# sanazkaviani/3d-latent-diffusion-model

Measured on AMD Instinct MI355X. Metric: UNet denoising steps/sec (bf16, 1x4x24x24x24 latent; whole job = sum over GPUs), higher is better.
Workload: dtype bf16

## Files before the change

3d-latent-diffusion-model_amd/csrc/attention.h:

```cpp
#pragma once
#include "common.h"

struct AttnParams {
    const bf16_t* qkv; bf16_t* out;
    int B, N, C, heads; float scale;
    float* lse;
    int d;
};

template <int S, int QW, bool DB, int D = 64>
__global__ __launch_bounds__(64 * QW * S) void attn_fwd_kernel(const AttnParams p) {
    constexpr int KT = 64;
    constexpr int NSL = (D + 63) / 64, DS = D < 64 ? D : 64;
    constexpr int K2 = DS / 32, NDT = DS / 16, CH = DS / 8;
    constexpr int IMG = KT * 128;
    constexpr int TILE = 2 * NSL * IMG;
    constexpr int GT = 64 * QW;
    constexpr int NIT = (KT * CH * NSL) / GT;
    static_assert(S == 1 || D == 64, "the in-workgroup key split is built for D = 64");
    static_assert((KT * CH * NSL) % GT == 0, "staging must divide evenly");
    extern __shared__ __attribute__((aligned(16))) char smem_all[];

    const int tid = threadIdx.x % GT, lane = tid & 63, wave = tid >> 6, grp = threadIdx.x / GT;
    char* smem = smem_all + grp * (DB ? 2 : 1) * TILE;
    const int fr = lane & 15, fg = lane >> 4;
    const int b = blockIdx.z, head = blockIdx.y;
    const int q0 = blockIdx.x * (16 * QW) + wave * 16;
    const int ld = 3 * p.C;
    const bf16_t* base = p.qkv + (size_t)b * p.N * ld;
    const int hoff = head * D;

    bf16x8 qf[NSL][K2];
    {
        int qr = q0 + fr; if (qr >= p.N) qr = p.N - 1;
#pragma unroll
        for (int sl = 0; sl < NSL; ++sl)
#pragma unroll
            for (int k2 = 0; k2 < K2; ++k2)
                qf[sl][k2] = *reinterpret_cast<const bf16x8*>(base + (size_t)qr * ld + hoff + sl * 64 + k2 * 32 + 8 * fg);
    }

    f32x4 ot[NSL][NDT];
#pragma unroll
    for (int sl = 0; sl < NSL; ++sl)
#pragma unroll
        for (int i = 0; i < NDT; ++i) ot[sl][i] = (f32x4){0.f, 0.f, 0.f, 0.f};
    float mrun = -INFINITY, lrun = 0.f;
    const float cexp = p.scale * 1.44269504088896340736f;

    u32x4 kreg[NIT], vreg[NIT];
    auto stage_load = [&](int k0) {
#pragma unroll
        for (int it = 0; it < NIT; ++it) {
            const int idx = tid + it * GT;
            const int sl = idx / (KT * CH), rem = idx - sl * (KT * CH);
            const int row = rem / CH, ch = rem - row * CH;
            int kr = k0 + row; if (kr >= p.N) kr = p.N - 1;
            const bf16_t* tok = base + (size_t)kr * ld + hoff + sl * 64 + ch * 8;
            kreg[it] = *reinterpret_cast<const u32x4*>(tok + p.C);
            vreg[it] = *reinterpret_cast<const u32x4*>(tok + 2 * p.C);
        }
    };
    auto stage_write = [&](char* ks, char* vs) {
#pragma unroll
        for (int it = 0; it < NIT; ++it) {
            const int idx = tid + it * GT;
            const int sl = idx / (KT * CH), rem = idx - sl * (KT * CH);
            const int row = rem / CH, ch = rem - row * CH;
            *reinterpret_cast<u32x4*>(ks + sl * IMG + row * 128 + ((ch ^ ((row >> 1) & 7)) << 4)) = kreg[it];
            *reinterpret_cast<u32x4*>(vs + sl * IMG + row * 128 + ((ch ^ (((row >> 1) & 3) << 1)) << 4)) = vreg[it];
        }
    };

    const int ntile = (p.N + KT - 1) / KT;
    const int nrounds = (ntile + S - 1) / S;
    stage_load(grp * KT);
#pragma unroll
    for (int sl = 0; sl < NSL; ++sl)
#pragma unroll
        for (int k2 = 0; k2 < K2; ++k2) asm volatile("" :: "v"(qf[sl][k2]));
    stage_write(smem, smem + NSL * IMG);
    __syncthreads();
    for (int it = 0; it < nrounds; ++it) {
        const int t = it * S + grp;
        const int k0 = t * KT;
        const char* ks = smem + (DB ? (it & 1) * TILE : 0);
        const char* vs = ks + NSL * IMG;
        stage_load(k0 + S * KT);
        if (t < ntile) {
        f32x4 st[4];
#pragma unroll
        for (int j = 0; j < 4; ++j) {
            st[j] = (f32x4){0.f, 0.f, 0.f, 0.f};
            const int row = j * 16 + fr;
#pragma unroll
            for (int sl = 0; sl < NSL; ++sl)
#pragma unroll
                for (int k2 = 0; k2 < K2; ++k2) {
                    const int c = k2 * 4 + fg;
                    const bf16x8 kf = *reinterpret_cast<const bf16x8*>(ks + sl * IMG + row * 128 + ((c ^ ((row >> 1) & 7)) << 4));
                    st[j] = __builtin_amdgcn_mfma_f32_16x16x32_bf16(kf, qf[sl][k2], st[j], 0, 0, 0);
                }
        }
        if (k0 + KT > p.N) {
#pragma unroll
            for (int j = 0; j < 4; ++j)
#pragma unroll
                for (int r = 0; r < 4; ++r)
                    if (k0 + 16 * j + 4 * fg + r >= p.N) st[j][r] = -INFINITY;
        }
        float tmax = fmaxf(fmaxf(fmaxf(st[0][0], st[0][1]), fmaxf(st[0][2], st[0][3])), fmaxf(fmaxf(st[1][0], st[1][1]), fmaxf(st[1][2], st[1][3])));
        tmax = fmaxf(tmax, fmaxf(fmaxf(fmaxf(st[2][0], st[2][1]), fmaxf(st[2][2], st[2][3])), fmaxf(fmaxf(st[3][0], st[3][1]), fmaxf(st[3][2], st[3][3]))));
        tmax = fmaxf(tmax, __shfl_xor(tmax, 16, 64));
        tmax = fmaxf(tmax, __shfl_xor(tmax, 32, 64));
        const float mnew = fmaxf(mrun, tmax);
        const float alpha = __builtin_amdgcn_exp2f((mrun - mnew) * cexp);
        const float mc = -mnew * cexp;
        mrun = mnew;
        float psum = 0.f;
        bf16x8 pf[2];
#pragma unroll
        for (int h = 0; h < 2; ++h) {
            float pv[8];
#pragma unroll
            for (int e = 0; e < 8; ++e) {
                const float pe = __builtin_amdgcn_exp2f(fmaf(st[2 * h + (e >> 2)][e & 3], cexp, mc));
                psum += pe;
                pv[e] = pe;
            }
            u32x4 pk;
#pragma unroll
            for (int e = 0; e < 4; ++e) pk[e] = pack2bf(pv[2 * e], pv[2 * e + 1]);
            pf[h] = *reinterpret_cast<bf16x8*>(&pk);
        }
        lrun = lrun * alpha + psum;
        if (__builtin_amdgcn_ballot_w64(alpha != 1.0f)) {
#pragma unroll
            for (int sl = 0; sl < NSL; ++sl)
#pragma unroll
                for (int dt = 0; dt < NDT; ++dt) {
#pragma unroll
                    for (int r = 0; r < 4; ++r) ot[sl][dt][r] *= alpha;
                }
        }
        typedef __attribute__((ext_vector_type(4))) short s16x4;
        typedef __attribute__((address_space(3))) s16x4* lds_s16x4_t;
        const int tq = fr >> 2, tp = fr & 3;
#pragma unroll
        for (int sl = 0; sl < NSL; ++sl)
#pragma unroll
        for (int dt = 0; dt < NDT; ++dt) {
#pragma unroll
            for (int h = 0; h < 2; ++h) {
                const int rlo = (2 * h) * 16 + 4 * fg + tq, rhi = rlo + 16;
                const char* alo = vs + sl * IMG + rlo * 128 + ((dt ^ ((rlo >> 1) & 3)) << 5) + tp * 8;
                const char* ahi = vs + sl * IMG + rhi * 128 + ((dt ^ ((rhi >> 1) & 3)) << 5) + tp * 8;
                const s16x4 lo = __builtin_amdgcn_ds_read_tr16_b64_v4i16((lds_s16x4_t)alo);
                const s16x4 hi = __builtin_amdgcn_ds_read_tr16_b64_v4i16((lds_s16x4_t)ahi);
                const bf16x8 vf = {lo[0], lo[1], lo[2], lo[3], hi[0], hi[1], hi[2], hi[3]};
                ot[sl][dt] = __builtin_amdgcn_mfma_f32_16x16x32_bf16(vf, pf[h], ot[sl][dt], 0, 0, 0);
            }
        }
        }
        if constexpr (!DB) __syncthreads();
        {
            char* nk = smem + (DB ? ((it + 1) & 1) * TILE : 0);
            stage_write(nk, nk + NSL * IMG);
        }
        __syncthreads();
    }
    lrun += __shfl_xor(lrun, 16, 64);
    lrun += __shfl_xor(lrun, 32, 64);
    if constexpr (S > 1) {
        float* xo = reinterpret_cast<float*>(smem_all) + (size_t)(grp * QW + wave) * (1024 + 32);
        if (grp > 0) {
#pragma unroll
            for (int dt = 0; dt < NDT; ++dt) *reinterpret_cast<f32x4*>(xo + (dt * 64 + lane) * 4) = ot[0][dt];
            if (fg == 0) { xo[1024 + fr] = mrun; xo[1040 + fr] = lrun; }
        }
        __syncthreads();
        if (grp > 0) return;
#pragma unroll
        for (int g = 1; g < S; ++g) {
            const float* xg = reinterpret_cast<const float*>(smem_all) + (size_t)(g * QW + wave) * (1024 + 32);
            const float mg = xg[1024 + fr], lg = xg[1040 + fr];
            const float mnew = fmaxf(mrun, mg);
            const float a0 = __builtin_amdgcn_exp2f((mrun - mnew) * cexp), a1 = __builtin_amdgcn_exp2f((mg - mnew) * cexp);
            lrun = lrun * a0 + lg * a1;
            mrun = mnew;
#pragma unroll
            for (int dt = 0; dt < NDT; ++dt) {
                const f32x4 og = *reinterpret_cast<const f32x4*>(xg + (dt * 64 + lane) * 4);
#pragma unroll
                for (int r = 0; r < 4; ++r) ot[0][dt][r] = ot[0][dt][r] * a0 + og[r] * a1;
            }
        }
    }
    const float inv = 1.0f / lrun;
    const int qr = q0 + fr;
    if (p.lse && qr < p.N && fg == 0) p.lse[((size_t)b * p.heads + head) * p.N + qr] = mrun * p.scale + __logf(lrun);
    if (qr < p.N) {
        bf16_t* orow = p.out + ((size_t)b * p.N + qr) * p.C + hoff;
#pragma unroll
        for (int sl = 0; sl < NSL; ++sl)
#pragma unroll
        for (int dt = 0; dt < NDT; ++dt) {
            u32x2 o;
            o[0] = pack2bf(ot[sl][dt][0] * inv, ot[sl][dt][1] * inv);
            o[1] = pack2bf(ot[sl][dt][2] * inv, ot[sl][dt][3] * inv);
            *reinterpret_cast<u32x2*>(orow + sl * 64 + dt * 16 + 4 * fg) = o;
        }
    }
}

template <int D>
static inline hipError_t launch_attn_fwd_d(const AttnParams& p, hipStream_t s) {
    constexpr int LDS = 2 * 2 * ((D + 63) / 64) * 64 * 128;
    static bool once_tab[32] = {}; bool& once = attr_flag(once_tab);
    if (!once) {
        hipError_t e = hipFuncSetAttribute(reinterpret_cast<const void*>(&attn_fwd_kernel<1, 4, true, D>), hipFuncAttributeMaxDynamicSharedMemorySize, LDS);
        if (e != hipSuccess) return e;
        once = true;
    }
    hipLaunchKernelGGL((attn_fwd_kernel<1, 4, true, D>), dim3((p.N + 63) / 64, p.heads, p.B), dim3(256), LDS, s, p);
    return hipGetLastError();
}
static inline hipError_t launch_attn_fwd(const AttnParams& p, hipStream_t s) {
    if (p.d == 32) return launch_attn_fwd_d<32>(p, s);
    if (p.d == 128) return launch_attn_fwd_d<128>(p, s);
    if (p.d == 256) return launch_attn_fwd_d<256>(p, s);
    if (p.d != 64) return hipErrorInvalidValue;
    static bool once_tab[32] = {}; bool& once = attr_flag(once_tab);
    if (!once) {
        hipError_t e = hipFuncSetAttribute(reinterpret_cast<const void*>(&attn_fwd_kernel<4, 4, true>), hipFuncAttributeMaxDynamicSharedMemorySize, 4 * 32768);
        if (e == hipSuccess) e = hipFuncSetAttribute(reinterpret_cast<const void*>(&attn_fwd_kernel<8, 2, false>), hipFuncAttributeMaxDynamicSharedMemorySize, 8 * 16384);
        if (e != hipSuccess) return e;
        once = true;
    }
    if (p.N >= 1024 && (long)((p.N + 63) / 64) * p.heads * p.B < 128)
        hipLaunchKernelGGL((attn_fwd_kernel<8, 2, false>), dim3((p.N + 31) / 32, p.heads, p.B), dim3(1024), 8 * 16384, s, p);
    else if (p.N > 3 * 64) hipLaunchKernelGGL((attn_fwd_kernel<4, 4, true>), dim3((p.N + 63) / 64, p.heads, p.B), dim3(1024), 4 * 32768, s, p);
    else hipLaunchKernelGGL((attn_fwd_kernel<1, 4, true>), dim3((p.N + 63) / 64, p.heads, p.B), dim3(256), 32768, s, p);
    return hipGetLastError();
}


struct AttnBwdParams {
    const bf16_t* qkv; const bf16_t* o; const bf16_t* d_o; const float* lse;
    float* delta;
    bf16_t* dqkv;
    int B, N, C, heads; float scale;
    int d;
};

__global__ __launch_bounds__(256) void attn_delta_kernel(const AttnBwdParams p) {
    const long idx = (long)blockIdx.x * 256 + threadIdx.x;
    const int cpd = p.d >> 3;
    const long total = (long)p.B * p.N * p.heads * cpd;
    float s = 0.f;
    long tok = 0; int head = 0;
    if (idx < total) {
        const int ch = (int)(idx % cpd);
        const long th = idx / cpd;
        head = (int)(th % p.heads); tok = th / p.heads;
        const u32x4 a = *reinterpret_cast<const u32x4*>(p.o + tok * p.C + head * p.d + ch * 8);
        const u32x4 b = *reinterpret_cast<const u32x4*>(p.d_o + tok * p.C + head * p.d + ch * 8);
#pragma unroll
        for (int k = 0; k < 4; ++k)
            s += __uint_as_float(a[k] << 16) * __uint_as_float(b[k] << 16) +
                 __uint_as_float(a[k] & 0xffff0000u) * __uint_as_float(b[k] & 0xffff0000u);
    }
    for (int o = 1; o < cpd; o <<= 1) s += __shfl_xor(s, o, 64);
    if (idx < total && (idx % cpd) == 0) {
        const long bb = tok / p.N, i = tok - bb * p.N;
        p.delta[((size_t)bb * p.heads + head) * p.N + i] = s;
    }
}

typedef __attribute__((ext_vector_type(4))) short attn_s16x4;
typedef __attribute__((address_space(3))) attn_s16x4* attn_lds_s16x4_t;

__device__ __forceinline__ int attn_row_off(int row, int ch) { return row * 128 + ((ch ^ ((row >> 1) & 7)) << 4); }
__device__ __forceinline__ int attn_tr_off(int row, int ch) { return row * 128 + ((ch ^ (((row >> 1) & 3) << 1)) << 4); }
__device__ __forceinline__ bf16x8 attn_tr_frag(const char* img, int dt, int h, int fr, int fg) {
    const int tq = fr >> 2, tp = fr & 3;
    const int rlo = (2 * h) * 16 + 4 * fg + tq, rhi = rlo + 16;
    const attn_s16x4 lo = __builtin_amdgcn_ds_read_tr16_b64_v4i16((attn_lds_s16x4_t)(img + rlo * 128 + ((dt ^ ((rlo >> 1) & 3)) << 5) + tp * 8));
    const attn_s16x4 hi = __builtin_amdgcn_ds_read_tr16_b64_v4i16((attn_lds_s16x4_t)(img + rhi * 128 + ((dt ^ ((rhi >> 1) & 3)) << 5) + tp * 8));
    return (bf16x8){lo[0], lo[1], lo[2], lo[3], hi[0], hi[1], hi[2], hi[3]};
}

template <int D>
__global__ __launch_bounds__(256) void attn_bwd_dq_kernel(const AttnBwdParams p) {
    constexpr int KT = 64;
    constexpr int NSL = (D + 63) / 64, DS = D < 64 ? D : 64, K2 = DS / 32, NDT = DS / 16, CH = DS / 8, IMG = KT * 128;
    constexpr int NIT = (KT * CH * NSL) / 256;
    extern __shared__ __attribute__((aligned(16))) char smem[];
    char* k_row = smem; char* k_tr = smem + NSL * IMG; char* v_row = smem + 2 * NSL * IMG;
    const int tid = threadIdx.x, lane = tid & 63, wave = tid >> 6;
    const int fr = lane & 15, fg = lane >> 4;
    const int b = blockIdx.z, head = blockIdx.y;
    const int q0 = blockIdx.x * 64 + wave * 16;
    const int ld = 3 * p.C, hoff = head * D;
    const bf16_t* base = p.qkv + (size_t)b * p.N * ld;
    int qr = q0 + fr; const bool qok = qr < p.N; if (!qok) qr = p.N - 1;
    bf16x8 qf[NSL][K2], dof[NSL][K2];
#pragma unroll
    for (int sl = 0; sl < NSL; ++sl)
#pragma unroll
    for (int k2 = 0; k2 < K2; ++k2) {
        qf[sl][k2] = *reinterpret_cast<const bf16x8*>(base + (size_t)qr * ld + hoff + sl * 64 + k2 * 32 + 8 * fg);
        dof[sl][k2] = *reinterpret_cast<const bf16x8*>(p.d_o + ((size_t)b * p.N + qr) * p.C + hoff + sl * 64 + k2 * 32 + 8 * fg);
    }
    const float lse = p.lse[((size_t)b * p.heads + head) * p.N + qr];
    const float dlt = p.delta[((size_t)b * p.heads + head) * p.N + qr];
    f32x4 dq[NSL][NDT];
#pragma unroll
    for (int sl = 0; sl < NSL; ++sl)
#pragma unroll
    for (int i = 0; i < NDT; ++i) dq[sl][i] = (f32x4){0.f, 0.f, 0.f, 0.f};
    const int ntile = (p.N + KT - 1) / KT;
    u32x4 kreg[NIT], vreg[NIT];
    auto stage_load = [&](int k0) {
#pragma unroll
        for (int it = 0; it < NIT; ++it) {
            const int idx = tid + it * 256, sl = idx / (KT * CH), rem = idx - sl * (KT * CH), row = rem / CH, ch = rem - row * CH;
            int kr = k0 + row; if (kr >= p.N) kr = p.N - 1;
            const bf16_t* tok = base + (size_t)kr * ld + hoff + sl * 64 + ch * 8;
            kreg[it] = *reinterpret_cast<const u32x4*>(tok + p.C);
            vreg[it] = *reinterpret_cast<const u32x4*>(tok + 2 * p.C);
        }
    };
    stage_load(0);
#pragma unroll
    for (int sl = 0; sl < NSL; ++sl)
#pragma unroll
        for (int k2 = 0; k2 < K2; ++k2) asm volatile("" :: "v"(qf[sl][k2]), "v"(dof[sl][k2]));
    asm volatile("" :: "v"(lse), "v"(dlt));
    for (int t = 0; t < ntile; ++t) {
        const int k0 = t * KT;
        __syncthreads();
#pragma unroll
        for (int it = 0; it < NIT; ++it) {
            const int idx = tid + it * 256, sl = idx / (KT * CH), rem = idx - sl * (KT * CH), row = rem / CH, ch = rem - row * CH;
            *reinterpret_cast<u32x4*>(k_row + sl * IMG + attn_row_off(row, ch)) = kreg[it];
            *reinterpret_cast<u32x4*>(k_tr + sl * IMG + attn_tr_off(row, ch)) = kreg[it];
            *reinterpret_cast<u32x4*>(v_row + sl * IMG + attn_row_off(row, ch)) = vreg[it];
        }
        __syncthreads();
        stage_load(k0 + KT);
        bf16x8 dsf[2];
        f32x4 st[4], dp[4];
#pragma unroll
        for (int j = 0; j < 4; ++j) {
            st[j] = (f32x4){0.f, 0.f, 0.f, 0.f}; dp[j] = (f32x4){0.f, 0.f, 0.f, 0.f};
            const int row = j * 16 + fr;
#pragma unroll
            for (int sl = 0; sl < NSL; ++sl)
#pragma unroll
            for (int k2 = 0; k2 < K2; ++k2) {
                const bf16x8 kf = *reinterpret_cast<const bf16x8*>(k_row + sl * IMG + attn_row_off(row, k2 * 4 + fg));
                const bf16x8 vf = *reinterpret_cast<const bf16x8*>(v_row + sl * IMG + attn_row_off(row, k2 * 4 + fg));
                st[j] = __builtin_amdgcn_mfma_f32_16x16x32_bf16(kf, qf[sl][k2], st[j], 0, 0, 0);
                dp[j] = __builtin_amdgcn_mfma_f32_16x16x32_bf16(vf, dof[sl][k2], dp[j], 0, 0, 0);
            }
        }
#pragma unroll
        for (int h = 0; h < 2; ++h) {
            float dsv[8];
#pragma unroll
            for (int e = 0; e < 8; ++e) {
                const int j = 2 * h + (e >> 2), r = e & 3;
                const int key = k0 + 16 * j + 4 * fg + r;
                const float pe = (key < p.N) ? __expf(st[j][r] * p.scale - lse) : 0.f;
                dsv[e] = pe * (dp[j][r] - dlt);
            }
            u32x4 pk;
#pragma unroll
            for (int e = 0; e < 4; ++e) pk[e] = pack2bf(dsv[2 * e], dsv[2 * e + 1]);
            dsf[h] = *reinterpret_cast<bf16x8*>(&pk);
        }
#pragma unroll
        for (int sl = 0; sl < NSL; ++sl)
#pragma unroll
        for (int dt = 0; dt < NDT; ++dt)
#pragma unroll
            for (int h = 0; h < 2; ++h)
                dq[sl][dt] = __builtin_amdgcn_mfma_f32_16x16x32_bf16(attn_tr_frag(k_tr + sl * IMG, dt, h, fr, fg), dsf[h], dq[sl][dt], 0, 0, 0);
    }
    if (qok) {
        bf16_t* orow = p.dqkv + ((size_t)b * p.N + qr) * ld + hoff;
#pragma unroll
        for (int sl = 0; sl < NSL; ++sl)
#pragma unroll
        for (int dt = 0; dt < NDT; ++dt) {
            u32x2 o;
            o[0] = pack2bf(dq[sl][dt][0] * p.scale, dq[sl][dt][1] * p.scale);
            o[1] = pack2bf(dq[sl][dt][2] * p.scale, dq[sl][dt][3] * p.scale);
            *reinterpret_cast<u32x2*>(orow + sl * 64 + dt * 16 + 4 * fg) = o;
        }
    }
}

template <int D>
__global__ __launch_bounds__(256) void attn_bwd_dkv_kernel(const AttnBwdParams p) {
    constexpr int QT = 64;
    constexpr int NSL = (D + 63) / 64, DS = D < 64 ? D : 64, K2 = DS / 32, NDT = DS / 16, CH = DS / 8, IMG = QT * 128;
    constexpr int NIT = (QT * CH * NSL) / 256;
    extern __shared__ __attribute__((aligned(16))) char smem[];
    char* q_row = smem; char* q_tr = smem + NSL * IMG; char* do_row = smem + 2 * NSL * IMG; char* do_tr = smem + 3 * NSL * IMG;
    float* s_lse = reinterpret_cast<float*>(smem + 4 * NSL * IMG); float* s_dlt = s_lse + QT;
    const int tid = threadIdx.x, lane = tid & 63, wave = tid >> 6;
    const int fr = lane & 15, fg = lane >> 4;
    const int b = blockIdx.z, head = blockIdx.y;
    const int kv0 = blockIdx.x * 64 + wave * 16;
    const int ld = 3 * p.C, hoff = head * D;
    const bf16_t* base = p.qkv + (size_t)b * p.N * ld;
    int kr = kv0 + fr; const bool kok = kr < p.N; if (!kok) kr = p.N - 1;
    bf16x8 kf[NSL][K2], vf[NSL][K2];
#pragma unroll
    for (int sl = 0; sl < NSL; ++sl)
#pragma unroll
    for (int k2 = 0; k2 < K2; ++k2) {
        kf[sl][k2] = *reinterpret_cast<const bf16x8*>(base + (size_t)kr * ld + p.C + hoff + sl * 64 + k2 * 32 + 8 * fg);
        vf[sl][k2] = *reinterpret_cast<const bf16x8*>(base + (size_t)kr * ld + 2 * p.C + hoff + sl * 64 + k2 * 32 + 8 * fg);
    }
    f32x4 dk[NSL][NDT], dv[NSL][NDT];
#pragma unroll
    for (int sl = 0; sl < NSL; ++sl)
#pragma unroll
    for (int i = 0; i < NDT; ++i) { dk[sl][i] = (f32x4){0.f, 0.f, 0.f, 0.f}; dv[sl][i] = (f32x4){0.f, 0.f, 0.f, 0.f}; }
    const int ntile = (p.N + QT - 1) / QT;
    u32x4 qreg[NIT], oreg[NIT]; float lreg = 0.f, dreg = 0.f;
    auto stage_load = [&](int q0) {
#pragma unroll
        for (int it = 0; it < NIT; ++it) {
            const int idx = tid + it * 256, sl = idx / (QT * CH), rem = idx - sl * (QT * CH), row = rem / CH, ch = rem - row * CH;
            int qr = q0 + row; if (qr >= p.N) qr = p.N - 1;
            qreg[it] = *reinterpret_cast<const u32x4*>(base + (size_t)qr * ld + hoff + sl * 64 + ch * 8);
            oreg[it] = *reinterpret_cast<const u32x4*>(p.d_o + ((size_t)b * p.N + qr) * p.C + hoff + sl * 64 + ch * 8);
        }
        {
            int qr = q0 + (tid & (QT - 1)); const bool ok = qr < p.N; if (!ok) qr = p.N - 1;
            const float l = p.lse[((size_t)b * p.heads + head) * p.N + qr];
            lreg = ok ? l : INFINITY;
            dreg = p.delta[((size_t)b * p.heads + head) * p.N + qr];
        }
    };
    stage_load(0);
#pragma unroll
    for (int sl = 0; sl < NSL; ++sl)
#pragma unroll
        for (int k2 = 0; k2 < K2; ++k2) asm volatile("" :: "v"(kf[sl][k2]), "v"(vf[sl][k2]));
    for (int t = 0; t < ntile; ++t) {
        const int q0 = t * QT;
        __syncthreads();
#pragma unroll
        for (int it = 0; it < NIT; ++it) {
            const int idx = tid + it * 256, sl = idx / (QT * CH), rem = idx - sl * (QT * CH), row = rem / CH, ch = rem - row * CH;
            *reinterpret_cast<u32x4*>(q_row + sl * IMG + attn_row_off(row, ch)) = qreg[it];
            *reinterpret_cast<u32x4*>(q_tr + sl * IMG + attn_tr_off(row, ch)) = qreg[it];
            *reinterpret_cast<u32x4*>(do_row + sl * IMG + attn_row_off(row, ch)) = oreg[it];
            *reinterpret_cast<u32x4*>(do_tr + sl * IMG + attn_tr_off(row, ch)) = oreg[it];
        }
        if (tid < QT) { s_lse[tid] = lreg; s_dlt[tid] = dreg; }
        __syncthreads();
        stage_load(q0 + QT);
        f32x4 st[4], dp[4];
#pragma unroll
        for (int j = 0; j < 4; ++j) {
            st[j] = (f32x4){0.f, 0.f, 0.f, 0.f}; dp[j] = (f32x4){0.f, 0.f, 0.f, 0.f};
            const int row = j * 16 + fr;
#pragma unroll
            for (int sl = 0; sl < NSL; ++sl)
#pragma unroll
            for (int k2 = 0; k2 < K2; ++k2) {
                const bf16x8 qf = *reinterpret_cast<const bf16x8*>(q_row + sl * IMG + attn_row_off(row, k2 * 4 + fg));
                const bf16x8 of = *reinterpret_cast<const bf16x8*>(do_row + sl * IMG + attn_row_off(row, k2 * 4 + fg));
                st[j] = __builtin_amdgcn_mfma_f32_16x16x32_bf16(qf, kf[sl][k2], st[j], 0, 0, 0);
                dp[j] = __builtin_amdgcn_mfma_f32_16x16x32_bf16(of, vf[sl][k2], dp[j], 0, 0, 0);
            }
        }
        bf16x8 pf[2], dsf[2];
#pragma unroll
        for (int h = 0; h < 2; ++h) {
            float pv[8], dsv[8];
#pragma unroll
            for (int e = 0; e < 8; ++e) {
                const int j = 2 * h + (e >> 2), r = e & 3;
                const int ql = 16 * j + 4 * fg + r;
                const float pe = __expf(st[j][r] * p.scale - s_lse[ql]);
                pv[e] = pe; dsv[e] = pe * (dp[j][r] - s_dlt[ql]);
            }
            u32x4 pk, dk_;
#pragma unroll
            for (int e = 0; e < 4; ++e) { pk[e] = pack2bf(pv[2 * e], pv[2 * e + 1]); dk_[e] = pack2bf(dsv[2 * e], dsv[2 * e + 1]); }
            pf[h] = *reinterpret_cast<bf16x8*>(&pk); dsf[h] = *reinterpret_cast<bf16x8*>(&dk_);
        }
#pragma unroll
        for (int sl = 0; sl < NSL; ++sl)
#pragma unroll
        for (int dt = 0; dt < NDT; ++dt)
#pragma unroll
            for (int h = 0; h < 2; ++h) {
                dv[sl][dt] = __builtin_amdgcn_mfma_f32_16x16x32_bf16(attn_tr_frag(do_tr + sl * IMG, dt, h, fr, fg), pf[h], dv[sl][dt], 0, 0, 0);
                dk[sl][dt] = __builtin_amdgcn_mfma_f32_16x16x32_bf16(attn_tr_frag(q_tr + sl * IMG, dt, h, fr, fg), dsf[h], dk[sl][dt], 0, 0, 0);
            }
    }
    if (kok) {
        bf16_t* orow = p.dqkv + ((size_t)b * p.N + kr) * ld + hoff;
#pragma unroll
        for (int sl = 0; sl < NSL; ++sl)
#pragma unroll
        for (int dt = 0; dt < NDT; ++dt) {
            u32x2 o;
            o[0] = pack2bf(dk[sl][dt][0] * p.scale, dk[sl][dt][1] * p.scale); o[1] = pack2bf(dk[sl][dt][2] * p.scale, dk[sl][dt][3] * p.scale);
            *reinterpret_cast<u32x2*>(orow + p.C + sl * 64 + dt * 16 + 4 * fg) = o;
            o[0] = pack2bf(dv[sl][dt][0], dv[sl][dt][1]); o[1] = pack2bf(dv[sl][dt][2], dv[sl][dt][3]);
            *reinterpret_cast<u32x2*>(orow + 2 * p.C + sl * 64 + dt * 16 + 4 * fg) = o;
        }
    }
}

template <int D>
static inline hipError_t launch_attn_bwd_d(const AttnBwdParams& p, hipStream_t s) {
    constexpr int NSL = (D + 63) / 64;
    constexpr int LDS_DQ = 3 * NSL * 64 * 128, LDS_DKV = 4 * NSL * 64 * 128 + 2 * 64 * 4;
    static bool once_tab[32] = {}; bool& once = attr_flag(once_tab);
    if (!once) {
        hipError_t e = hipFuncSetAttribute(reinterpret_cast<const void*>(&attn_bwd_dq_kernel<D>), hipFuncAttributeMaxDynamicSharedMemorySize, LDS_DQ);
        if (e == hipSuccess) e = hipFuncSetAttribute(reinterpret_cast<const void*>(&attn_bwd_dkv_kernel<D>), hipFuncAttributeMaxDynamicSharedMemorySize, LDS_DKV);
        if (e != hipSuccess) return e;
        once = true;
    }
    const long dthreads = (long)p.B * p.N * p.heads * (D / 8);
    hipLaunchKernelGGL(attn_delta_kernel, dim3((unsigned)((dthreads + 255) / 256)), dim3(256), 0, s, p);
    hipLaunchKernelGGL(attn_bwd_dq_kernel<D>, dim3((p.N + 63) / 64, p.heads, p.B), dim3(256), LDS_DQ, s, p);
    hipLaunchKernelGGL(attn_bwd_dkv_kernel<D>, dim3((p.N + 63) / 64, p.heads, p.B), dim3(256), LDS_DKV, s, p);
    return hipGetLastError();
}
static inline hipError_t launch_attn_bwd(const AttnBwdParams& p, hipStream_t s) {
    switch (p.d) {
        case 32: return launch_attn_bwd_d<32>(p, s);
        case 64: return launch_attn_bwd_d<64>(p, s);
        case 128: return launch_attn_bwd_d<128>(p, s);
        case 256: return launch_attn_bwd_d<256>(p, s);
    }
    return hipErrorInvalidValue;
}
```

Before: 515.7.

## Add DMA-to-LDS ring-buffered attention forward kernel for long low-occupancy sequences

Result: no change. 520.7 (median of 6 runs) (+1.0%).

```diff
diff --git a/3d-latent-diffusion-model_amd/csrc/attention.h b/3d-latent-diffusion-model_amd/csrc/attention.h
--- a/3d-latent-diffusion-model_amd/csrc/attention.h
+++ b/3d-latent-diffusion-model_amd/csrc/attention.h
@@ -213,6 +213,253 @@
     }
 }
 
+constexpr __host__ __device__ int attn_dma_swz(bool v_img, int row) { return v_img ? ((row >> 1) & 3) << 1 : (row >> 1) & 7; }
+constexpr __host__ __device__ int attn_dma_src_chunk(bool v_img, int row, int slot) { return slot ^ attn_dma_swz(v_img, row); }
+constexpr bool attn_dma_map_ok(bool v_img) {
+    for (int row = 0; row < 64; ++row) {
+        unsigned seen = 0;
+        for (int slot = 0; slot < 8; ++slot) {
+            const int ch = attn_dma_src_chunk(v_img, row, slot);
+            if (ch < 0 || ch > 7) return false;
+            seen |= 1u << ch;
+            const int rd = v_img ? (ch ^ (((row >> 1) & 3) << 1)) : (ch ^ ((row >> 1) & 7));
+            if (rd != slot) return false;
+        }
+        if (seen != 0xffu) return false;
+    }
+    return true;
+}
+static_assert(attn_dma_map_ok(false) && attn_dma_map_ok(true), "slot -> source map must be a bijection and the inverse of the read-side swizzle");
+
+typedef __attribute__((ext_vector_type(4))) short attn_dma_s16x4;
+__device__ __forceinline__ attn_dma_s16x4 attn_dma_read_tr(unsigned lds_addr) {
+    attn_dma_s16x4 v;
+    asm volatile("ds_read_b64_tr_b16 %0, %1" : "=v"(v) : "v"(lds_addr));
+    return v;
+}
+
+template <int S, int QW, int R>
+__global__ __launch_bounds__(64 * QW * S) void attn_fwd_dma_kernel(const AttnParams p) {
+#if defined(__HIP_DEVICE_COMPILE__)
+    constexpr int KT = 64, IMG = KT * 128, TILE = 2 * IMG, GT = 64 * QW;
+    constexpr int PW = 16 / QW;
+    constexpr unsigned OOB = 0x80000000u;
+    static_assert(QW == 2 || QW == 4, "16 pieces per tile are dealt evenly to the group's waves");
+    static_assert(R >= 2 && (R & (R - 1)) == 0 && (R - 1) * PW <= 63, "ring depth: a power of two; vmcnt is a 6-bit counter");
+    static_assert(S * R * TILE <= 160 * 1024 && S * QW * (1024 + 32) * 4 <= S * R * TILE, "LDS budget; the merge area reuses the rings");
+    typedef __attribute__((address_space(3))) void* lds_ptr_t;
+    extern __shared__ __attribute__((aligned(16))) char smem_all[];
+    KSTAMP_BEGIN(8);
+
+    const int tid = threadIdx.x % GT, lane = tid & 63;
+    const int wave = __builtin_amdgcn_readfirstlane(tid >> 6), grp = __builtin_amdgcn_readfirstlane(threadIdx.x / GT);
+    char* smem = smem_all + grp * (R * TILE);
+    const int fr = lane & 15, fg = lane >> 4;
+    const int b = blockIdx.z, head = blockIdx.y;
+    const int q0 = blockIdx.x * (16 * QW) + wave * 16;
+    const int ld = 3 * p.C;
+    const int hoff = head * 64;
+    const int ntile = (p.N + KT - 1) / KT;
+    const int nrounds = (ntile + S - 1) / S;
+
+    bf16x8 qf[2];
+    {
+        int qr = q0 + fr; if (qr >= p.N) qr = p.N - 1;
+        const bf16_t* qrow = p.qkv + ((size_t)b * p.N + qr) * ld + hoff;
+#pragma unroll
+        for (int k2 = 0; k2 < 2; ++k2) qf[k2] = *reinterpret_cast<const bf16x8*>(qrow + k2 * 32 + 8 * fg);
+    }
+
+    const __amdgpu_buffer_rsrc_t rs = __builtin_amdgcn_make_buffer_rsrc((void*)p.qkv, 0, (int)((unsigned)(p.B * p.N) * (unsigned)ld * 2u), 0x00020000);
+    const unsigned ld2 = (unsigned)ld * 2u, tok0 = (unsigned)(b * p.N);
+    int c_row[PW]; unsigned c_col[PW];
+#pragma unroll
+    for (int j = 0; j < PW; ++j) {
+        const int pc = wave * PW + j;
+        const bool v_img = pc >= 8;
+        const int row = (pc & 7) * 8 + (lane >> 3);
+        c_row[j] = row;
+        c_col[j] = (unsigned)((v_img ? 2 : 1) * p.C + hoff + attn_dma_src_chunk(v_img, row, lane & 7) * 8) * 2u;
+    }
+    auto issue = [&](const int i) {
+        const int t = i * S + grp, k0 = t * KT;
+        char* dst = smem + (i & (R - 1)) * TILE + wave * (PW * 1024);
+        const unsigned oob = t < ntile ? 0u : OOB;
+#pragma unroll
+        for (int j = 0; j < PW; ++j) {
+            int kr = k0 + c_row[j]; if (kr >= p.N) kr = p.N - 1;
+            const unsigned vo = ((tok0 + (unsigned)kr) * ld2 + c_col[j]) | oob;
+            __builtin_amdgcn_raw_ptr_buffer_load_lds(rs, (lds_ptr_t)(dst + j * 1024), 16, vo, 0, 0, 0);
+        }
+    };
+#pragma unroll
+    for (int i = 0; i < R - 1; ++i) issue(i);
+#pragma unroll
+    for (int k2 = 0; k2 < 2; ++k2) asm volatile("" :: "v"(qf[k2]));
+    KSTAMP(1);
+
+    f32x4 ot[4];
+#pragma unroll
+    for (int i = 0; i < 4; ++i) ot[i] = (f32x4){0.f, 0.f, 0.f, 0.f};
+    float mrun = -INFINITY, lrun = 0.f;
+    const float cexp = p.scale * 1.44269504088896340736f;
+
+    int k_off[4][2];
+#pragma unroll
+    for (int j = 0; j < 4; ++j)
+#pragma unroll
+        for (int k2 = 0; k2 < 2; ++k2) {
+            const int row = j * 16 + fr, c = k2 * 4 + fg;
+            k_off[j][k2] = row * 128 + ((c ^ ((row >> 1) & 7)) << 4);
+        }
+    unsigned v_lo[4][2], v_hi[4][2];
+    {
+        const int tq = fr >> 2, tp = fr & 3;
+        const unsigned sbase = (unsigned)(size_t)(const __attribute__((address_space(3))) char*)smem + IMG;
+#pragma unroll
+        for (int dt = 0; dt < 4; ++dt)
+#pragma unroll
+            for (int h = 0; h < 2; ++h) {
+                const int rlo = (2 * h) * 16 + 4 * fg + tq, rhi = rlo + 16;
+                v_lo[dt][h] = sbase + rlo * 128 + ((dt ^ ((rlo >> 1) & 3)) << 5) + tp * 8;
+                v_hi[dt][h] = sbase + rhi * 128 + ((dt ^ ((rhi >> 1) & 3)) << 5) + tp * 8;
+            }
+    }
+
+    for (int it = 0; it < nrounds; ++it) {
+        asm volatile("s_waitcnt vmcnt(%0)" ::"n"((R - 2) * PW) : "memory");
+        asm volatile("s_waitcnt lgkmcnt(0)" ::: "memory");
+        __builtin_amdgcn_s_barrier();
+        asm volatile("" ::: "memory");
+        __builtin_amdgcn_sched_barrier(0);
+        if (it == 0) KSTAMP(2);
+        issue(it + R - 1);
+        const int t = it * S + grp, k0 = t * KT;
+        if (t < ntile) {
+            const int soff = (it & (R - 1)) * TILE;
+            const char* ks = smem + soff;
+            f32x4 st[4];
+#pragma unroll
+            for (int j = 0; j < 4; ++j) {
+                st[j] = (f32x4){0.f, 0.f, 0.f, 0.f};
+#pragma unroll
+                for (int k2 = 0; k2 < 2; ++k2) {
+                    const bf16x8 kf = *reinterpret_cast<const bf16x8*>(ks + k_off[j][k2]);
+                    st[j] = __builtin_amdgcn_mfma_f32_16x16x32_bf16(kf, qf[k2], st[j], 0, 0, 0);
+                }
+            }
+            attn_dma_s16x4 vl[4][2], vh[4][2];
+#pragma unroll
+            for (int dt = 0; dt < 4; ++dt)
+#pragma unroll
+                for (int h = 0; h < 2; ++h) {
+                    vl[dt][h] = attn_dma_read_tr(v_lo[dt][h] + soff);
+                    vh[dt][h] = attn_dma_read_tr(v_hi[dt][h] + soff);
+                }
+            if (k0 + KT > p.N) {
+#pragma unroll
+                for (int j = 0; j < 4; ++j)
+#pragma unroll
+                    for (int r = 0; r < 4; ++r)
+                        if (k0 + 16 * j + 4 * fg + r >= p.N) st[j][r] = -INFINITY;
+            }
+            float tmax = fmaxf(fmaxf(fmaxf(st[0][0], st[0][1]), fmaxf(st[0][2], st[0][3])), fmaxf(fmaxf(st[1][0], st[1][1]), fmaxf(st[1][2], st[1][3])));
+            tmax = fmaxf(tmax, fmaxf(fmaxf(fmaxf(st[2][0], st[2][1]), fmaxf(st[2][2], st[2][3])), fmaxf(fmaxf(st[3][0], st[3][1]), fmaxf(st[3][2], st[3][3]))));
+            tmax = fmaxf(tmax, __shfl_xor(tmax, 16, 64));
+            tmax = fmaxf(tmax, __shfl_xor(tmax, 32, 64));
+            const float mnew = fmaxf(mrun, tmax);
+            const float alpha = __builtin_amdgcn_exp2f((mrun - mnew) * cexp);
+            const float mc = -mnew * cexp;
+            mrun = mnew;
+            float psum = 0.f;
+            bf16x8 pf[2];
+#pragma unroll
+            for (int h = 0; h < 2; ++h) {
+                float pv[8];
+#pragma unroll
+                for (int e = 0; e < 8; ++e) {
+                    const float pe = __builtin_amdgcn_exp2f(fmaf(st[2 * h + (e >> 2)][e & 3], cexp, mc));
+                    psum += pe;
+                    pv[e] = pe;
+                }
+                u32x4 pk;
+#pragma unroll
+                for (int e = 0; e < 4; ++e) pk[e] = pack2bf(pv[2 * e], pv[2 * e + 1]);
+                pf[h] = *reinterpret_cast<bf16x8*>(&pk);
+            }
+            lrun = lrun * alpha + psum;
+            if (__builtin_amdgcn_ballot_w64(alpha != 1.0f)) {
+#pragma unroll
+                for (int dt = 0; dt < 4; ++dt)
+#pragma unroll
+                    for (int r = 0; r < 4; ++r) ot[dt][r] *= alpha;
+            }
+            asm volatile("s_waitcnt lgkmcnt(0)"
+                         : "+v"(vl[0][0]), "+v"(vl[0][1]), "+v"(vl[1][0]), "+v"(vl[1][1]), "+v"(vl[2][0]), "+v"(vl[2][1]), "+v"(vl[3][0]), "+v"(vl[3][1]),
+                           "+v"(vh[0][0]), "+v"(vh[0][1]), "+v"(vh[1][0]), "+v"(vh[1][1]), "+v"(vh[2][0]), "+v"(vh[2][1]), "+v"(vh[3][0]), "+v"(vh[3][1])
+                         :: "memory");
+#pragma unroll
+            for (int dt = 0; dt < 4; ++dt)
+#pragma unroll
+                for (int h = 0; h < 2; ++h) {
+                    const bf16x8 vf = {vl[dt][h][0], vl[dt][h][1], vl[dt][h][2], vl[dt][h][3], vh[dt][h][0], vh[dt][h][1], vh[dt][h][2], vh[dt][h][3]};
+                    ot[dt] = __builtin_amdgcn_mfma_f32_16x16x32_bf16(vf, pf[h], ot[dt], 0, 0, 0);
+                }
+        }
+    }
+    asm volatile("s_waitcnt vmcnt(0) lgkmcnt(0)" ::: "memory");
+    KSTAMP(3);
+    lrun += __shfl_xor(lrun, 16, 64);
+    lrun += __shfl_xor(lrun, 32, 64);
+    if constexpr (S > 1) {
+        __syncthreads();
+        float* xo = reinterpret_cast<float*>(smem_all) + (size_t)(grp * QW + wave) * (1024 + 32);
+        if (grp > 0) {
+#pragma unroll
+            for (int dt = 0; dt < 4; ++dt) *reinterpret_cast<f32x4*>(xo + (dt * 64 + lane) * 4) = ot[dt];
+            if (fg == 0) { xo[1024 + fr] = mrun; xo[1040 + fr] = lrun; }
+        }
+        __syncthreads();
+        if (grp > 0) return;
+#pragma unroll
+        for (int g = 1; g < S; ++g) {
+            const float* xg = reinterpret_cast<const float*>(smem_all) + (size_t)(g * QW + wave) * (1024 + 32);
+            const float mg = xg[1024 + fr], lg = xg[1040 + fr];
+            const float mnew = fmaxf(mrun, mg);
+            const float a0 = __builtin_amdgcn_exp2f((mrun - mnew) * cexp), a1 = __builtin_amdgcn_exp2f((mg - mnew) * cexp);
+            lrun = lrun * a0 + lg * a1;
+            mrun = mnew;
+#pragma unroll
+            for (int dt = 0; dt < 4; ++dt) {
+                const f32x4 og = *reinterpret_cast<const f32x4*>(xg + (dt * 64 + lane) * 4);
+#pragma unroll
+                for (int r = 0; r < 4; ++r) ot[dt][r] = ot[dt][r] * a0 + og[r] * a1;
+            }
+        }
+    }
+    KSTAMP(4);
+    const float inv = 1.0f / lrun;
+    const int qr = q0 + fr;
+    if (p.lse && qr < p.N && fg == 0) p.lse[((size_t)b * p.heads + head) * p.N + qr] = mrun * p.scale + __logf(lrun);
+    if (qr < p.N) {
+        bf16_t* orow = p.out + ((size_t)b * p.N + qr) * p.C + hoff;
+#pragma unroll
+        for (int dt = 0; dt < 4; ++dt) {
+            u32x2 o;
+            o[0] = pack2bf(ot[dt][0] * inv, ot[dt][1] * inv);
+            o[1] = pack2bf(ot[dt][2] * inv, ot[dt][3] * inv);
+            *reinterpret_cast<u32x2*>(orow + dt * 16 + 4 * fg) = o;
+        }
+    }
+    KSTAMP_DRAIN(5);
+#endif
+}
+
+template <int S, int QW, int R>
+static inline void launch_attn_fwd_dma(const AttnParams& p, hipStream_t s) {
+    hipLaunchKernelGGL((attn_fwd_dma_kernel<S, QW, R>), dim3((p.N + 16 * QW - 1) / (16 * QW), p.heads, p.B), dim3(64 * QW * S), S * R * 16384, s, p);
+}
+
 template <int D>
 static inline hipError_t launch_attn_fwd_d(const AttnParams& p, hipStream_t s) {
     constexpr int LDS = 2 * 2 * ((D + 63) / 64) * 64 * 128;
@@ -234,12 +481,27 @@
     if (!once) {
         hipError_t e = hipFuncSetAttribute(reinterpret_cast<const void*>(&attn_fwd_kernel<4, 4, true>), hipFuncAttributeMaxDynamicSharedMemorySize, 4 * 32768);
         if (e == hipSuccess) e = hipFuncSetAttribute(reinterpret_cast<const void*>(&attn_fwd_kernel<8, 2, false>), hipFuncAttributeMaxDynamicSharedMemorySize, 8 * 16384);
+        if (e == hipSuccess) e = hipFuncSetAttribute(reinterpret_cast<const void*>(&attn_fwd_dma_kernel<4, 2, 2>), hipFuncAttributeMaxDynamicSharedMemorySize, 8 * 16384);
+#ifdef LDM_EXPERIMENTS
+        if (e == hipSuccess) e = hipFuncSetAttribute(reinterpret_cast<const void*>(&attn_fwd_dma_kernel<2, 4, 4>), hipFuncAttributeMaxDynamicSharedMemorySize, 8 * 16384);
+        if (e == hipSuccess) e = hipFuncSetAttribute(reinterpret_cast<const void*>(&attn_fwd_dma_kernel<1, 4, 8>), hipFuncAttributeMaxDynamicSharedMemorySize, 8 * 16384);
+#endif
         if (e != hipSuccess) return e;
         once = true;
     }
-    if (p.N >= 1024 && (long)((p.N + 63) / 64) * p.heads * p.B < 128)
-        hipLaunchKernelGGL((attn_fwd_kernel<8, 2, false>), dim3((p.N + 31) / 32, p.heads, p.B), dim3(1024), 8 * 16384, s, p);
-    else if (p.N > 3 * 64) hipLaunchKernelGGL((attn_fwd_kernel<4, 4, true>), dim3((p.N + 63) / 64, p.heads, p.B), dim3(1024), 4 * 32768, s, p);
+    if (p.N >= 1024 && (long)((p.N + 63) / 64) * p.heads * p.B < 128) {
+        if (ldm_knob("LDM_ATTN_DMA", 1) == 0)
+            hipLaunchKernelGGL((attn_fwd_kernel<8, 2, false>), dim3((p.N + 31) / 32, p.heads, p.B), dim3(1024), 8 * 16384, s, p);
+        else {
+#ifdef LDM_EXPERIMENTS
+            const long cfg = ldm_xknob("LDM_ATTN_DMA_CFG", 0);
+            if (cfg == 1) launch_attn_fwd_dma<2, 4, 4>(p, s);
+            else if (cfg == 2) launch_attn_fwd_dma<1, 4, 8>(p, s);
+            else
+#endif
+            launch_attn_fwd_dma<4, 2, 2>(p, s);
+        }
+    } else if (p.N > 3 * 64) hipLaunchKernelGGL((attn_fwd_kernel<4, 4, true>), dim3((p.N + 63) / 64, p.heads, p.B), dim3(1024), 4 * 32768, s, p);
     else hipLaunchKernelGGL((attn_fwd_kernel<1, 4, true>), dim3((p.N + 63) / 64, p.heads, p.B), dim3(256), 32768, s, p);
     return hipGetLastError();
 }
```
